# mazpie/genrl

Measured on AMD Instinct MI355X. Metric: world-model+imag update steps/sec (B32xL32x64x64x3), higher is better.
Workload: dtype f32 (storage, accumulation, every non-GEMM kernel and the fp32-MFMA GEMMs; the forward / dgrad / weight-gradient products of the imagination rollout, of the Dense+LN+SiLU chains from 192 rows up and of the encoder / decoder convolutions take fp32 operands pre-split into two fp16 planes of the scaled

## Files before the change

### genrl_amd/csrc/gemm_planes.hip

```cpp
#include "common.h"
#include "genrl_hip.h"
#include <type_traits>

typedef __bf16 bf16x8_t __attribute__((ext_vector_type(8)));
typedef _Float16 f16x8_t __attribute__((ext_vector_type(8)));
typedef unsigned u32x4 __attribute__((ext_vector_type(4)));

namespace {

struct PlaneSeg {
  const u16* a; long a_ld, a_plane;
  const u16* b; long b_ld, b_plane;
  int k;
  const float* a_inv; const float* b_inv;
};

struct SampleEpi {
  const float* q;
  long ldq;
  float* sample; long lds;
  u16* sp; long sld, splane; float* sinv;
  float a;
};

// ... 9 lines not shown
  float eps; int act;
  float* y; long ldy;
  u16* yp; long yld, yplane; float* yinv;
  float* mean; float* rstd;
  float* part;
  unsigned* sync;
};

struct PairSel {
  const u16* b; long b_ld, b_plane; const float* b_inv;
  float* C; long ldc; int N, accumulate;
  int tn0, nx;
};

__device__ __forceinline__ float pow2_ratio(float a, float b) {
  const int ea = (int)((__builtin_bit_cast(unsigned, a) >> 23) & 255u), eb = (int)((__builtin_bit_cast(unsigned, b) >> 23) & 255u);
  const int e = min(max(ea - eb + 127, 1), 254);
  return __builtin_bit_cast(float, (unsigned)e << 23);
}
__device__ __forceinline__ bool zero_row_inv(float inv) { return __builtin_bit_cast(unsigned, inv) == (4u << 23); }

__device__ __forceinline__ void glds16(const void* g, unsigned lds_byte_addr) {
  __builtin_amdgcn_global_load_lds((const __attribute__((address_space(1))) void*)g,
                                   (__attribute__((address_space(3))) void*)(uintptr_t)lds_byte_addr, 16, 0, 0);
}

template <int N> __device__ __forceinline__ void wait_vm() { asm volatile("s_waitcnt vmcnt(%0)" ::"i"(N) : "memory"); }

template <int TM, int TN, int BK, int NACC, int FMT, int NS, bool FOLD, bool CONV, int PF, bool LNE, bool IS_PAIR>
__device__ __forceinline__ void gemm_planes_body(PlaneSeg s0, PlaneSeg s1, float* __restrict__ C, long ldc,
                                                 const float* __restrict__ bias, int M, int N, int accumulate,
                                                 int tiles_m, int tiles_n, int xcd_m, SampleEpi smp, ConvGather cg, LnEpi ln, PairSel pr) {
  static_assert(!LNE || (TM * TN == 1 && FMT == 1 && !CONV && PF == 0), "LayerNorm epilogue: 64x64 h2 tile");
  static_assert(!IS_PAIR || (TM * TN == 1 && FMT == 1 && !CONV && PF == 0 && !LNE), "pair of products: 64x64 h2 tile");
  constexpr int BM = 64 * TM, BN = 64 * TN;
  static_assert(!(FMT == 1 && FOLD) || (BM == 64 && BN == 64), "segment fold: 64x64 h2 tile");
  constexpr int NPL = FMT ? 2 : 3, NPROD = FMT ? 3 : 6;
  constexpr int ROWB = BK * 2;
  constexpr int CPR = ROWB / 16;
  constexpr int RPC = 1024 / ROWB;
  constexpr int A_BYTES = NPL * BM * ROWB, B_BYTES = NPL * BN * ROWB, STAGE = A_BYTES + B_BYTES;
  constexpr int APIECES = A_BYTES / 1024, BPIECES = B_BYTES / 1024;
  static_assert(APIECES % 2 == 0 && BPIECES % 2 == 0, "pieces split over two waves per operand");
  constexpr int NPA = APIECES / 2, NPB = BPIECES / 2;
  constexpr int NPMAX = NPA > NPB ? NPA : NPB;
  constexpr int KS = BK / 16;
  static_assert(PF == 0 || (BK == 64 && !CONV), "prefetch: 128-byte tile rows, plain operands");
  constexpr int NPF = PF ? TM : 0;
  constexpr int EPI = FMT == 1 ? 4 * (BM + 2 * BN) : 0, EPI_AT = NS * STAGE + (PF ? 1024 : 0);
  constexpr int LN_AT = EPI_AT + EPI, LN_G = LN_AT, LN_B = LN_AT + 4096, LN_R = LN_AT + 8192, LN_U = LN_AT + 9216, LN_T = LN_AT + 9472, LN_BYTES = LNE ? 9728 : 0;
  __shared__ __attribute__((aligned(1024))) unsigned char lds[EPI_AT + EPI + LN_BYTES];

  int bid = blockIdx.x, tile_m, tile_n;
  {
    const int ntiles = tiles_m * tiles_n;
    int x = bid % 8;
    const int i = bid / 8;
    if constexpr (LNE) {
      unsigned xcc;
      asm volatile("s_getreg_b32 %0, hwreg(HW_REG_XCC_ID)" : "=s"(xcc));
      x = (int)(xcc & 7u);
      tile_n = i % tiles_n; tile_m = (i / tiles_n) * 8 + x;
      if (tile_m >= tiles_m) return;
    } else if (xcd_m > 0) {
      const int sub_m = tiles_m / xcd_m, sub_n = tiles_n / (8 / xcd_m);
      const int xm = x / (8 / xcd_m), xn = x % (8 / xcd_m);
      tile_m = xm * sub_m + i / sub_n;
      tile_n = xn * sub_n + i % sub_n;
    } else {
      const int q = ntiles / 8, r = ntiles % 8;
      bid = (x < r ? x * (q + 1) : r * (q + 1) + (x - r) * q) + i;
      tile_m = bid / tiles_n;
      tile_n = bid % tiles_n;
    }
  }
  if constexpr (IS_PAIR) {
    const int tn1 = tiles_n - pr.tn0;
    bool second;
    if (pr.nx > 0) {
      const int sub_n = tiles_n / pr.nx, q0 = pr.tn0 / pr.nx, xn = tile_n / sub_n, jn = tile_n % sub_n;
      second = jn >= q0;
      tile_n = second ? xn * (tn1 / pr.nx) + jn - q0 : xn * q0 + jn;
    } else {
      second = tile_n >= pr.tn0;
      if (second) tile_n -= pr.tn0;
    }
    if (second) {
      s0.b = pr.b; s0.b_ld = pr.b_ld; s0.b_plane = pr.b_plane; s0.b_inv = pr.b_inv;
      C = pr.C; ldc = pr.ldc; N = pr.N; accumulate = pr.accumulate;
    }
  }
  const int m0 = tile_m * BM, n0 = tile_n * BN;
  const int tid = threadIdx.x, lane = tid & 63;
  const int wave = __builtin_amdgcn_readfirstlane(tid >> 6);
  const int wm = wave >> 1, wn = wave & 1;
  const unsigned lds0 = (unsigned)(uintptr_t)lds;

  const bool isB = wave >= 2;
  const int npieces = isB ? NPB : NPA;
  const int rows_t = isB ? BN : BM;
  const int gpp = rows_t / RPC;
  const int r_in = lane / CPR, slot = lane % CPR;
  const char* gbase;
  unsigned voff[NPMAX];
  unsigned pfoff[NPF ? NPF : 1];
  auto setup = [&](const PlaneSeg& s) __attribute__((always_inline)) {
    const u16* P = isB ? s.b : s.a;
    const long ld = isB ? s.b_ld : s.a_ld, plane = isB ? s.b_plane : s.a_plane;
    const int rows_total = isB ? N : M, r0 = isB ? n0 : m0;
    gbase = reinterpret_cast<const char*>(P);
    if constexpr (PF > 0) {
#pragma unroll
      for (int i = 0; i < NPF; ++i) {
        const int L = ((wave & 1) * NPF + i) * 64 + lane;
        const int p = L / rows_t, row = L % rows_t;
        pfoff[i] = (unsigned)((p * plane + (long)min(r0 + row, rows_total - 1) * ld) * 2);
      }
    }
#pragma unroll
    for (int i = 0; i < NPMAX; ++i) {
      const int q = (wave & 1) * npieces + i;
      const int p = q / gpp, row = (q % gpp) * RPC + r_in;
      const int f = BK == 64 ? (row >> 1) & 7 : (row >> 2) & 3;
      voff[i] = (unsigned)((p * plane + (long)min(r0 + row, rows_total - 1) * ld) * 2 + ((slot ^ f) << 4));
    }
  };
  unsigned koff[2] = {0u, 0u};
  int kch[2] = {0, 0}, kkw[2] = {0, 0}, kkk[2] = {0, 0};
  if constexpr (CONV) {
    if (!isB) {
      const long ld = s0.a_ld, plane = s0.a_plane;
      gbase = reinterpret_cast<const char*>(s0.a);
#pragma unroll
      for (int i = 0; i < NPMAX; ++i) {
        const int q = (wave & 1) * npieces + i;
        const int p = q / gpp, row = (q % gpp) * RPC + r_in;
        const int m = min(m0 + row, M - 1);
        const int n_img = m / (cg.Ho * cg.Wo), rem = m - n_img * (cg.Ho * cg.Wo);
        const int oy = rem / cg.Wo, ox = rem - oy * cg.Wo;
        voff[i] = (unsigned)(((long)p * plane + ((long)(n_img * cg.H + cg.s * oy) * cg.W + cg.s * ox) * ld) * 2);
      }
#pragma unroll
      for (int par = 0; par < 2; ++par) {
        const int f = (4 * par + (r_in >> 1)) & 7;
        const int kk = 8 * (slot ^ f);
        const int tap = kk / cg.C, ch = kk - tap * cg.C, kh = tap / cg.k, kw = tap - kh * cg.k;
        kkk[par] = kk; kch[par] = ch; kkw[par] = kw;
        koff[par] = (unsigned)((((long)kh * cg.W + kw) * ld + ch) * 2);
      }
    }
  }
  const unsigned piece0 = lds0 + (isB ? A_BYTES : 0) + (wave & 1) * npieces * 1024;
  const int l32 = lane & 31, h32 = lane >> 5;
  const int f_rd = BK == 64 ? (l32 >> 1) & 7 : (l32 >> 2) & 3;
  unsigned xoff[KS];
#pragma unroll
  for (int s = 0; s < KS; ++s) xoff[s] = (unsigned)(((2 * s + h32) ^ f_rd) << 4);
  const unsigned a_row = lds0 + (wm * 32 * TM + l32) * ROWB, b_row = lds0 + A_BYTES + (wn * 32 * TN + l32) * ROWB;

  f32x16 acc[NACC][TM][TN];
#pragma unroll
  for (int c = 0; c < NACC; ++c)
#pragma unroll
    for (int i = 0; i < TM; ++i)
#pragma unroll
      for (int j = 0; j < TN; ++j)
#pragma unroll
        for (int r = 0; r < 16; ++r) acc[c][i][j][r] = 0.f;

  auto ldfrag = [&](unsigned addr) __attribute__((always_inline)) -> u32x4 {
    return *reinterpret_cast<const __attribute__((address_space(3))) u32x4*>((uintptr_t)addr);
  };
  constexpr int NB_ = TM + TN, NR = KS * NB_ * NPL, NM = KS * NPROD * TM * TN;
  constexpr int KB = 2;
  u32x4 fr[2][KS][NB_][NPL];
  unsigned a_s[KS], b_s[KS];
#pragma unroll
  for (int s = 0; s < KS; ++s) { a_s[s] = a_row + xoff[s]; b_s[s] = b_row + xoff[s]; }
  auto read_one = [&](int set, int r, int buf) __attribute__((always_inline)) {
    const int s = r / (NB_ * NPL), p = (r / NB_) % NPL, blk = r % NB_;
    fr[set][s][blk][p] = blk < TM ? ldfrag(a_s[s] + (p * (BM * ROWB) + blk * 32 * ROWB + buf * STAGE))
                                  : ldfrag(b_s[s] + (p * (BN * ROWB) + (blk - TM) * 32 * ROWB + buf * STAGE));
  };
  auto mfma_one = [&](int set, int m) __attribute__((always_inline)) {
    constexpr int PA[6] = {FMT ? 1 : 2, FMT ? 0 : 1, 0, 0, 1, 0}, PB[6] = {0, 0, FMT ? 1 : 2, 0, 1, 1};
// ... 3 lines not shown
    if constexpr (FMT == 0)
      c = __builtin_amdgcn_mfma_f32_32x32x16_bf16(__builtin_bit_cast(bf16x8_t, fr[set][s][TM + j][PB[t]]),
                                                  __builtin_bit_cast(bf16x8_t, fr[set][s][i][PA[t]]), c, 0, 0, 0);
    else
      c = __builtin_amdgcn_mfma_f32_32x32x16_f16(__builtin_bit_cast(f16x8_t, fr[set][s][TM + j][PB[t]]),
                                                 __builtin_bit_cast(f16x8_t, fr[set][s][i][PA[t]]), c, 0, 0, 0);
  };

  const float* const ainv_l = s1.k ? s1.a_inv : s0.a_inv;
  const float* const binv_l = s1.k ? s1.b_inv : s0.b_inv;
  if constexpr (FMT == 1) {
    const float* src = wave == 0 ? ainv_l : (wave == 1 ? binv_l : (wave == 2 ? bias : nullptr));
    const int base = wave == 0 ? m0 : n0, lim = (wave == 0 ? M : N) - 1, cnt = (wave == 0 ? BM : BN) / 64;
    const unsigned dst = lds0 + EPI_AT + (wave == 0 ? 0 : (wave == 1 ? 4 * BM : 4 * (BM + BN)));
    if (src) {
#pragma unroll
      for (int j = 0; j < (BM > BN ? BM : BN) / 64; ++j)
        if (j < cnt)
          __builtin_amdgcn_global_load_lds((const __attribute__((address_space(1))) void*)(src + min(base + 64 * j + lane, lim)),
                                           (__attribute__((address_space(3))) void*)(uintptr_t)(dst + 256 * j), 4, 0, 0);
    }
  }
  if constexpr (LNE) {
    const int f0 = min(256 * wave + 4 * lane, N - 4);
    __builtin_amdgcn_global_load_lds((const __attribute__((address_space(1))) void*)(ln.gamma + f0),
                                     (__attribute__((address_space(3))) void*)(uintptr_t)(lds0 + LN_G + 1024 * wave), 16, 0, 0);
    __builtin_amdgcn_global_load_lds((const __attribute__((address_space(1))) void*)(ln.beta + f0),
                                     (__attribute__((address_space(3))) void*)(uintptr_t)(lds0 + LN_B + 1024 * wave), 16, 0, 0);
    if (wave == 3)
      __builtin_amdgcn_global_load_lds((const __attribute__((address_space(1))) void*)(ln.part + ln_slab(tiles_n) + ((long)(tile_m * tiles_n + tile_n) * 64 + lane) * 4 + 1),
                                       (__attribute__((address_space(3))) void*)(uintptr_t)(lds0 + LN_T), 4, 0, 0);
  }
  const int nk0 = s0.k / BK, nk = nk0 + s1.k / BK;
  static_assert(NPA == NPB, "square wave grids only (one DMA count per wave)");
  constexpr int NP = NPA;
  if (!(CONV && !isB)) setup(s0);
  int seg_left = nk0, left = nk;
  bool first = true;
  auto next_stage = [&]() __attribute__((always_inline)) {
    if constexpr (CONV) {
      if (!isB) {
        if (!first && left > 0) {
          const unsigned ld2 = (unsigned)(s0.a_ld * 2);
#pragma unroll
          for (int par = 0; par < 2; ++par) {
            if (kkk[par] + 64 + 8 <= cg.K) {
              kkk[par] += 64;
              int ch = kch[par] + 64, kw = kkw[par];
              unsigned off = koff[par] + 128u;
#pragma unroll
              for (int rep = 0; rep < 2; ++rep)
                if (ch >= cg.C) {
                  ch -= cg.C; off -= (unsigned)(cg.C * 2);
                  ++kw; off += ld2;
                  if (kw == cg.k) { kw = 0; off += (unsigned)(cg.W - cg.k) * ld2; }
                }
              kch[par] = ch; kkw[par] = kw; koff[par] = off;
            }
          }
        }
        first = false;
        --seg_left; --left;
        return;
      }
    }
    if (seg_left == 0 && left > 0) { setup(s1); seg_left = left; }
    else if (!first && left > 0) gbase += BK * 2;
    first = false;
    --seg_left; --left;
  };
  auto prefetch = [&]() __attribute__((always_inline)) {
    if constexpr (PF > 0) {
      const int ahead = min(PF, max(seg_left, 0)) * (BK * 2);
#pragma unroll
      for (int i = 0; i < NPF; ++i)
        __builtin_amdgcn_global_load_lds((const __attribute__((address_space(1))) void*)(gbase + (size_t)pfoff[i] + ahead),
                                         (__attribute__((address_space(3))) void*)(uintptr_t)(lds0 + NS * STAGE + wave * 256), 4, 0, 0);
    }
  };
  auto issue_one = [&](int buf, int i) __attribute__((always_inline)) {
    if constexpr (CONV) {
      if (!isB) { glds16(gbase + (size_t)(voff[i] + koff[i & 1]), piece0 + buf * STAGE + i * 1024); return; }
    }
    glds16(gbase + (size_t)voff[i], piece0 + buf * STAGE + i * 1024);
  };
#pragma unroll
  for (int st = 0; st < NS; ++st) {
    next_stage();
    if (st) prefetch();
#pragma unroll
    for (int i = 0; i < NP; ++i) issue_one(st, i);
  }
  next_stage();
  wait_vm<(NS - 1) * (NP + NPF)>();
  __builtin_amdgcn_s_barrier();
#pragma unroll
  for (int r = 0; r < NR; ++r) read_one(0, r, 0);

  if constexpr (FMT == 1 && FOLD) {
    if (s1.k && wave < 2) {
      typedef __attribute__((address_space(3))) float lds_f32;
      lds_f32* const f = reinterpret_cast<lds_f32*>((uintptr_t)(lds0 + EPI_AT + 4 * (wave * BM + lane)));
      if ((wave ? s1.b_inv : s1.a_inv) && zero_row_inv(*f)) {
        const float* const inv0 = wave ? s0.b_inv : s0.a_inv;
        *f = inv0 ? inv0[min((wave ? n0 : m0) + lane, (wave ? N : M) - 1)] : 1.f;
      }
    }
  }
  auto epi1 = [&](int i) __attribute__((always_inline)) -> float {
    return *reinterpret_cast<const __attribute__((address_space(3))) float*>((uintptr_t)(lds0 + EPI_AT + 4 * i));
  };
  int it = 0;
  auto fold = [&]() __attribute__((always_inline)) {
    if constexpr (FMT == 1) {
#pragma unroll
      for (int i = 0; i < TM; ++i) {
        const int row = min(m0 + (wm * TM + i) * 32 + l32, M - 1);
        const int ri = (wm * TM + i) * 32 + l32;
        const float rf = (s0.a_inv && s1.a_inv) ? pow2_ratio(s0.a_inv[row], epi1(ri)) : (s0.a_inv ? s0.a_inv[row] : (s1.a_inv ? pow2_ratio(1.f, epi1(ri)) : 1.f));
#pragma unroll
        for (int j = 0; j < TN; ++j)
#pragma unroll
          for (int v = 0; v < 16; ++v) {
            const int col = min(n0 + (wn * TN + j) * 32 + 8 * (v / 4) + 4 * h32 + v % 4, N - 1);
            const int ci = BM + (wn * TN + j) * 32 + 8 * (v / 4) + 4 * h32 + v % 4;
            const float cf = (s0.b_inv && s1.b_inv) ? pow2_ratio(s0.b_inv[col], epi1(ci)) : (s0.b_inv ? s0.b_inv[col] : (s1.b_inv ? pow2_ratio(1.f, epi1(ci)) : 1.f));
#pragma unroll
            for (int c = 0; c < NACC; ++c) acc[c][i][j][v] *= rf * cf;
          }
      }
    }
  };

  constexpr int NSIDE = NP + NR;
  constexpr int PER = (NSIDE + 1) / 2 <= NM - KB - 2 ? 2 : 3;
  static_assert(NR >= 2 * NP, "side-op pattern: two reads per DMA");
  static_assert((NSIDE + PER - 1) / PER <= NM - KB - 2, "not enough MFMAs to hide the side operations");
  auto iteration = [&](auto SET, auto BUF) __attribute__((always_inline)) {
    constexpr int set = decltype(SET)::value, b0 = decltype(BUF)::value;
    constexpr int buf1 = (b0 + 1) % NS, buf3 = b0;
    if constexpr (FMT == 1 && FOLD) {
      if (it == nk0) fold();
    }
#pragma unroll
    for (int m = 0; m < KB; ++m) mfma_one(set, m);
    __builtin_amdgcn_sched_barrier(0);
    wait_vm<(NS - 2) * (NP + NPF)>();
    asm volatile("s_waitcnt lgkmcnt(0)" ::: "memory");
    __builtin_amdgcn_s_barrier();
    __builtin_amdgcn_sched_barrier(0);
    prefetch();
#pragma unroll
    for (int m = KB; m < NM; ++m) {
      mfma_one(set, m);
      const int lo = (m - KB) * PER, hi = lo + PER;
#pragma unroll
      for (int o = lo; o < hi; ++o) {
        if (o >= NSIDE) continue;
        if (o < 3 * NP && o % 3 == 2) {
          issue_one(buf3, o / 3);
        } else {
          read_one(1 - set, o < 3 * NP ? o - o / 3 : o - NP, buf1);
        }
      }
      __builtin_amdgcn_sched_barrier(0);
    }
    next_stage();
    ++it;
  };
  constexpr int PERIOD = NS % 2 ? 2 * NS : NS;
  auto run = [&](auto self, auto P, bool guarded) __attribute__((always_inline)) -> void {
    constexpr int p = decltype(P)::value;
    if constexpr (p < PERIOD) {
      if (guarded && it >= nk) return;
      iteration(std::integral_constant<int, p % 2>{}, std::integral_constant<int, p % NS>{});
      self(self, std::integral_constant<int, p + 1>{}, guarded);
    }
  };
  while (it + PERIOD <= nk) run(run, std::integral_constant<int, 0>{}, false);
  run(run, std::integral_constant<int, 0>{}, true);

  if constexpr (LNE) {
    typedef __attribute__((address_space(1))) unsigned gu32_;
    auto ldsf = [&](int byte_off) __attribute__((always_inline)) -> float {
      return *reinterpret_cast<const __attribute__((address_space(3))) float*>((uintptr_t)(lds0 + byte_off));
    };
    auto ldsw = [&](int byte_off, float v) __attribute__((always_inline)) {
      *reinterpret_cast<__attribute__((address_space(3))) float*>((uintptr_t)(lds0 + byte_off)) = v;
    };
    auto ldsf4 = [&](int byte_off) __attribute__((always_inline)) -> f32x4 {
      return *reinterpret_cast<const __attribute__((address_space(3))) f32x4*>((uintptr_t)(lds0 + byte_off));
    };
    const int rl = wm * 32 + l32, row = m0 + rl;
    const float ra = ainv_l ? ldsf(EPI_AT + 4 * rl) : 1.f;
    float o[16];
#pragma unroll
    for (int gq = 0; gq < 4; ++gq) {
      const int ci = wn * 32 + 8 * gq + 4 * h32;
      f32x4 cb = {1.f, 1.f, 1.f, 1.f}, bs = {0.f, 0.f, 0.f, 0.f};
      if (binv_l) cb = ldsf4(EPI_AT + 4 * (BM + ci));
      if (bias) bs = ldsf4(EPI_AT + 4 * (BM + BN + ci));
#pragma unroll
      for (int v = 0; v < 4; ++v) {
        const float lo = acc[0][0][0][4 * gq + v] + acc[2][0][0][4 * gq + v];
        o[4 * gq + v] = (lo * (1.f / 2048.f) + acc[1][0][0][4 * gq + v]) * ra * cb[v] + bs[v];
      }
    }
    float sm = 0.f;
#pragma unroll
    for (int v = 0; v < 16; ++v) sm += o[v];
    sm += __shfl_xor(sm, 32, 64);
    if (h32 == 0) ldsw(LN_R + 4 * (wave * 32 + l32), sm);
    __syncthreads();
// ... 1109 lines not shown
  for (int i = 0; i < n; ++i) {
    const int Co = d[i].transpose ? d[i].R : d[i].Cn;
    if (d[i].R <= 0 || d[i].Cn <= 0 || d[i].ld_out < Co || !d[i].inv || (d[i].ld_out & 63)) return GENRL_EINVAL;
  }
  hipStream_t s = (hipStream_t)stream;
  for (int pass = 0; pass < 2; ++pass) {
    int i = 0;
    while (i < n) {
      SplitBatch rows{}, cols{}, tiles{};
      int nb = 0;
      for (; i < n && nb < 32; ++i) {
        if ((d[i].transpose != 0) != (pass == 1)) continue;
        const SplitEntry e{d[i].src, d[i].ldx, d[i].R, d[i].Cn, d[i].out, d[i].ld_out, d[i].plane, d[i].inv};
        rows.e[nb] = cols.e[nb] = tiles.e[nb] = e;
        rows.blk0[nb + 1] = rows.blk0[nb] + cdiv(e.R, 4);
        cols.blk0[nb + 1] = cols.blk0[nb] + cdiv(e.Cn, 32);
        tiles.blk0[nb + 1] = tiles.blk0[nb] + cdiv(e.ld_out, 32) * cdiv(e.Cn, 32);
        ++nb;
      }
      if (!nb) continue;
      rows.n = cols.n = tiles.n = nb;
      if (pass == 0) {
        split_h2_rows_batch_kernel<<<rows.blk0[nb], 256, 0, s>>>(rows);
      } else {
        h2_colmax_batch_kernel<<<cols.blk0[nb], 256, 0, s>>>(cols);
        split_h2_t_batch_kernel<<<tiles.blk0[nb], 256, 0, s>>>(tiles);
      }
      GENRL_CHECK_LAUNCH();
    }
  }
  return GENRL_OK;
}

struct H2Route { bool big, two; };
static H2Route h2_route(int M, int N, int K, bool sample) {
  static const char* two_env = getenv("GENRL_PLANES_2PER");
  const long t64 = (long)cdiv(M, 64) * cdiv(N, 64);
  H2Route r;
  r.big = sample ? false : (g_planes_force_tile ? g_planes_force_tile == 2 : t64 >= 2048);
  r.two = !sample && (two_env ? two_env[0] == '1' : (t64 > 256 && K <= 1536));
  return r;
}

static int gemm_h2_impl(const uint16_t* a0, long a0_ld, long a0_plane, const float* a0_inv, const uint16_t* b0, long b0_ld, long b0_plane,
                        const float* b0_inv, int k0, const uint16_t* a1, long a1_ld, long a1_plane, const float* a1_inv,
                        const uint16_t* b1, long b1_ld, long b1_plane, const float* b1_inv, int k1,
                        float* C, long ldc, const float* bias, int M, int N, int accumulate, void* stream, const SampleEpi& smp) {
  GENRL_ENTER();
  if (M <= 0 || N <= 0 || k0 <= 0 || (k0 & 63) || (k1 & 63) || k1 < 0) return GENRL_EINVAL;
  if ((a0_ld & 7) || (b0_ld & 7) || (k1 && ((a1_ld & 7) || (b1_ld & 7)))) return GENRL_EINVAL;
  PlaneSeg s0{a0, a0_ld, a0_plane, b0, b0_ld, b0_plane, k0, a0_inv, b0_inv}, s1{a1, a1_ld, a1_plane, b1, b1_ld, b1_plane, k1, a1_inv, b1_inv};
  const H2Route rt = h2_route(M, N, k0 + k1, smp.q != nullptr);
  const bool big = rt.big;
  if (big && !g_planes_force_tile) {
    const int tm = cdiv(M, 128), tn = cdiv(N, 128), total = tm * tn, r = total % 256;
    if (total > 256 && r && r <= 128 && r % tn == 0 && (M & 127) == 0) {
      const int M1 = (tm - r / tn) * 128, M2 = M - M1;
      int rc = gemm_h2_impl(a0, a0_ld, a0_plane, a0_inv, b0, b0_ld, b0_plane, b0_inv, k0, a1, a1_ld, a1_plane, a1_inv, b1, b1_ld, b1_plane,
                            b1_inv, k1, C, ldc, bias, M1, N, accumulate, stream, smp);
      if (rc != GENRL_OK) return rc;
      return gemm_h2_impl(a0 + (long)M1 * a0_ld, a0_ld, a0_plane, a0_inv ? a0_inv + M1 : nullptr, b0, b0_ld, b0_plane, b0_inv, k0,
                          a1 ? a1 + (long)M1 * a1_ld : nullptr, a1_ld, a1_plane, a1_inv ? a1_inv + M1 : nullptr, b1, b1_ld, b1_plane, b1_inv, k1,
                          C + (long)M1 * ldc, ldc, bias, M2, N, accumulate, stream, smp);
    }
  }
  if (big) {
    const int tm = cdiv(M, 128), tn = cdiv(N, 128);
    const PlaneSeg none{nullptr, 0, 0, nullptr, 0, 0, 0, nullptr, nullptr};
    for (int seg = 0; seg < (k1 ? 2 : 1); ++seg) {
      const PlaneSeg& sg = seg ? s1 : s0;
      const float* bs = seg ? nullptr : bias;
      const int acc = seg ? 1 : accumulate;
      log_launch("h2/128", M, N, sg.k, kk_bytes(M, N, sg.k));
      route(!hl_on() ? GENRL_ROUTE_128_PLAIN : use_wide(N) ? GENRL_ROUTE_128_HLW : GENRL_ROUTE_128_HL);
      if (hl_on() && use_wide(N)) {
        const int tw = cdiv(N, 192);
        gemm_planes_hlw_kernel<false, 3><<<tm * tw, 256, 0, (hipStream_t)stream>>>(sg, C, ldc, bs, M, N, acc, tm, tw, xcd_split(tm, tw), ConvGather{});
      } else if (hl_on()) {
        gemm_planes_hl_kernel<false><<<tm * tn, 256, 0, (hipStream_t)stream>>>(sg, C, ldc, bs, M, N, acc, tm, tn, xcd_split(tm, tn) | (1 << 8), ConvGather{});
      } else
        gemm_planes_kernel<2, 2, 64, 2, 1, 2, false><<<tm * tn, 256, 0, (hipStream_t)stream>>>(sg, none, C, ldc, bs, M, N, acc, tm, tn,
                                                                                           xcd_split(tm, tn), SampleEpi{}, ConvGather{}, LnEpi{});
      GENRL_CHECK_LAUNCH();
    }
  } else {
    const int tm = cdiv(M, 64), tn = cdiv(N, 64);
    log_launch("h2/64", M, N, k0 + k1, kk_bytes(M, N, k0 + k1));
#define L64(NS_) gemm_planes_kernel<1, 1, 64, 3, 1, NS_, true><<<tm * tn, 256, 0, (hipStream_t)stream>>>( \
    s0, s1, C, ldc, bias, M, N, accumulate, tm, tn, xcd_split(tm, tn), smp, ConvGather{}, LnEpi{})
    const bool two = rt.two;
    route(smp.q ? GENRL_ROUTE_64_SAMPLE : (two ? GENRL_ROUTE_64_NS2 : GENRL_ROUTE_64_NS3));
    if (two) L64(2);
    else L64(3);
#undef L64
  }
  GENRL_CHECK_LAUNCH();
  return GENRL_OK;
}

int genrl_gemm_h2_conv(const uint16_t* img, long ld_img, long plane_img, const float* img_inv, int Nimg, int H, int W, int Cc, int k,
                       const uint16_t* b, long b_ld, long b_plane, const float* b_inv, float* C, long ldc, const float* bias, int N,
                       int accumulate, void* stream) {
  GENRL_ENTER();
  route_reset();
  const int Ho = (H - k) / 2 + 1, Wo = (W - k) / 2 + 1, K = k * k * Cc;
  const long Ml = (long)Nimg * Ho * Wo;
  if (Nimg <= 0 || Ho <= 0 || Wo <= 0 || N <= 0 || (Cc & 7) || Cc < 48 || ld_img < Cc || (ld_img & 7) || (b_ld & 63) || b_ld < K || b_ld >= K + 64 || K < 64 ||
      !img_inv || !b_inv || Ml > 0x7fffffffL)
    return GENRL_EINVAL;
  if ((((long)Nimg * H * W * ld_img + plane_img) * 2) >= 0xffffffffL) return GENRL_EINVAL;
  const int M = (int)Ml;
  PlaneSeg s0{img, ld_img, plane_img, b, b_ld, b_plane, (int)b_ld, img_inv, b_inv};
  const PlaneSeg none{nullptr, 0, 0, nullptr, 0, 0, 0, nullptr, nullptr};
  const bool wide = hl_on() && use_wide(N);
  const bool tall = hl_on() && use_tall96(N, K);
  const int tm = cdiv(M, tall ? 256 : 128), tn = tall ? 1 : cdiv(N, wide ? 192 : 128);
  log_launch("h2/conv128", M, N, (int)b_ld, 4.0 * ((double)Nimg * H * W * Cc + (double)N * b_ld + (double)M * N));
// ... 31 lines not shown
  const int M = (int)Ml;
  PlaneSeg s0{img, ld_img, plane_img, b, b_ld, b_plane, (int)b_ld, img_inv, b_inv};
  const bool wide = use_wide(N);
  const int tm = cdiv(M, 128), tn = cdiv(N, wide ? 192 : 128);
  log_launch("h2/subpixel128", M, N, (int)b_ld, 4.0 * ((double)Nimg * Hp * Wp * Cc + (double)N * b_ld + (double)Nimg * Ho * Wo * Co));
  route(wide ? GENRL_ROUTE_SUBPIXEL_HLW : GENRL_ROUTE_SUBPIXEL_HL);
  if (wide)
    gemm_planes_hlw_kernel<true, 3><<<tm * tn, 256, 0, (hipStream_t)stream>>>(s0, out, 4, bias, M, N, 0, tm, tn, xcd_split(tm, tn),
                                                                             ConvGather{Hp, Wp, Cc, T, Hq, Wq, K, 1, Ho, Wo, Co});
  else
    gemm_planes_hl_kernel<true><<<tm * tn, 256, 0, (hipStream_t)stream>>>(s0, out, 4, bias, M, N, 0, tm, tn, xcd_split(tm, tn),
                                                                          ConvGather{Hp, Wp, Cc, T, Hq, Wq, K, 1, Ho, Wo, Co});
  GENRL_CHECK_LAUNCH();
  return GENRL_OK;
}

int genrl_gemm_h2(const uint16_t* a0, long a0_ld, long a0_plane, const float* a0_inv, const uint16_t* b0, long b0_ld, long b0_plane,
                  const float* b0_inv, int k0, const uint16_t* a1, long a1_ld, long a1_plane, const float* a1_inv,
                  const uint16_t* b1, long b1_ld, long b1_plane, const float* b1_inv, int k1,
                  float* C, long ldc, const float* bias, int M, int N, int accumulate, void* stream) {
  route_reset();
  return gemm_h2_impl(a0, a0_ld, a0_plane, a0_inv, b0, b0_ld, b0_plane, b0_inv, k0, a1, a1_ld, a1_plane, a1_inv, b1, b1_ld, b1_plane,
                      b1_inv, k1, C, ldc, bias, M, N, accumulate, stream, SampleEpi{});
}

int genrl_gemm_h2_pair(const uint16_t* a, long a_ld, long a_plane, const float* a_inv, int k,
                       const uint16_t* b0, long b0_ld, long b0_plane, const float* b0_inv, float* C0, long ldc0, int N0, int accumulate0,
                       const uint16_t* b1, long b1_ld, long b1_plane, const float* b1_inv, float* C1, long ldc1, int N1, int accumulate1,
                       int M, void* stream) {
  GENRL_ENTER();
  route_reset();
  if (M <= 0 || N0 <= 0 || N1 <= 0 || k <= 0 || (k & 63) || (N0 & 63) || !a || !b0 || !b1 || !C0 || !C1) return GENRL_EINVAL;
  if ((a_ld & 7) || (b0_ld & 7) || (b1_ld & 7)) return GENRL_EINVAL;
  const int tm = cdiv(M, 64), tn0 = N0 / 64, tn1 = cdiv(N1, 64), tn = tn0 + tn1;
  for (int i = 0; i < 2; ++i) {
    const H2Route rt = h2_route(M, i ? N1 : N0, k, false);
    if (rt.big || rt.two) return GENRL_EINVAL;
  }
  const PlaneSeg s0{a, a_ld, a_plane, b0, b0_ld, b0_plane, k, a_inv, b0_inv};
  const int xm = xcd_split(tm, tn);
  const int nx = xm > 0 ? 8 / xm : 0;
  const PairSel pr{b1, b1_ld, b1_plane, b1_inv, C1, ldc1, N1, accumulate1, tn0, (nx > 0 && tn0 % nx == 0 && tn1 % nx == 0) ? nx : 0};
  log_launch("h2/64", M, (long)N0 + N1, k, kk_bytes(M, (long)N0 + N1, k));
  route(GENRL_ROUTE_64_NS3);
  gemm_planes_kernel<1, 1, 64, 3, 1, 3, PairOfProducts><<<tm * tn, 256, 0, (hipStream_t)stream>>>(s0, C0, ldc0, M, N0, accumulate0, tm, tn, xm, pr);
  GENRL_CHECK_LAUNCH();
  return GENRL_OK;
}

int genrl_gemm_h2_ln_ok(int M, int N) {
  if (M <= 0 || N <= 0 || (N & 63) || N > 1024) return 0;
  static int cus = -1;
  if (cus < 0) { int dev = 0, v = 0; if (hipGetDevice(&dev) != hipSuccess || hipDeviceGetAttribute(&v, hipDeviceAttributeMultiprocessorCount, dev) != hipSuccess) v = 0; cus = v; }
  if (cus < 256) return 0;
  const int tn = N / 64, tm = cdiv(M, 64);
  return tm <= 8 * (32 / tn) ? 1 : 0;
}
long genrl_gemm_h2_ln_part_floats(int M, int N) { (void)M; (void)N; return 16L * 65536; }
long genrl_gemm_h2_ln_sync_words(void) { return 32L; }
int genrl_gemm_h2_ln(const uint16_t* a0, long a0_ld, long a0_plane, const float* a0_inv, const uint16_t* b0, long b0_ld, long b0_plane,
                     const float* b0_inv, int k0, const uint16_t* a1, long a1_ld, long a1_plane, const float* a1_inv,
                     const uint16_t* b1, long b1_ld, long b1_plane, const float* b1_inv, int k1,
                     float* C, long ldc, const float* bias, int M, int N, const float* gamma, const float* beta, float eps, int act,
                     float* y, long ldy, float* mean, float* rstd, uint16_t* yp, long yld, long yplane, float* yinv,
                     float* part, unsigned* sync, void* stream) {
  GENRL_ENTER();
  route_reset();
  if (bad_act_code(act)) return GENRL_EINVAL;
  if (!genrl_gemm_h2_ln_ok(M, N) || k0 <= 0 || (k0 & 63) || (k1 & 63) || k1 < 0 || !gamma || !beta || !part || !sync || !C) return GENRL_EINVAL;
  if ((a0_ld & 7) || (b0_ld & 7) || (k1 && ((a1_ld & 7) || (b1_ld & 7))) || (ldc & 3) || (y && (ldy & 3)) || (yp && ((yld & 3) || !yinv))) return GENRL_EINVAL;
  if (((reinterpret_cast<uintptr_t>(C) | reinterpret_cast<uintptr_t>(bias) | reinterpret_cast<uintptr_t>(gamma) | reinterpret_cast<uintptr_t>(beta) |
        reinterpret_cast<uintptr_t>(y) | reinterpret_cast<uintptr_t>(part)) & 15) != 0 || (reinterpret_cast<uintptr_t>(yp) & 7) != 0)
    return GENRL_EINVAL;
  PlaneSeg s0{a0, a0_ld, a0_plane, b0, b0_ld, b0_plane, k0, a0_inv, b0_inv}, s1{a1, a1_ld, a1_plane, b1, b1_ld, b1_plane, k1, a1_inv, b1_inv};
  const int tm = cdiv(M, 64), tn = N / 64;
  const LnEpi ln{gamma, beta, eps, act, y, ldy, yp, yld, yplane, yinv, mean, rstd, part, sync};
  log_launch("h2/64ln", M, N, k0 + k1, kk_bytes(M, N, k0 + k1));
  route(GENRL_ROUTE_64_LN);
// ... 22 lines not shown
```

### include/genrl_hip.h

```cpp
#ifndef GENRL_HIP_H
#define GENRL_HIP_H
#include <stdint.h>
#ifdef __cplusplus
extern "C" {
#endif

long genrl_sgemm_ws_floats(int M, int N, int K);
int genrl_set_gemm_precision(int mode);
int genrl_sgemm_last_pipe(void);
int genrl_gemm_precision(void);
int genrl_sgemm(const float* A, long a_rs, long a_ks, const float* B, long b_rs, long b_ks, float* C, long ldc,
                const float* bias, int M, int N, int K, int accumulate, float* ws, long ws_floats, void* stream);

int genrl_sgemm_conv(const float* A, long a_rs, long a_ks, const float* B, long b_rs, long b_ks, float* C, long ldc,
                     const float* bias, int M, int N, int K, int accumulate, float* ws, long ws_floats, int which,
                     int img_h, int img_w, int img_c, int ksize, void* stream);

int genrl_split_h2(const float* x, long ldx, int R, int Cn, uint16_t* out, long ld_out, long plane, float* inv, int transpose,
                   void* stream);
int genrl_gemm_h2(const uint16_t* a0, long a0_ld, long a0_plane, const float* a0_inv, const uint16_t* b0, long b0_ld, long b0_plane,
                  const float* b0_inv, int k0, const uint16_t* a1, long a1_ld, long a1_plane, const float* a1_inv,
                  const uint16_t* b1, long b1_ld, long b1_plane, const float* b1_inv, int k1,
                  float* C, long ldc, const float* bias, int M, int N, int accumulate, void* stream);
int genrl_gemm_h2_pair(const uint16_t* a, long a_ld, long a_plane, const float* a_inv, int k,
// ... 126 lines not shown
int genrl_gemm_h2_tn_conv(const uint16_t* a, long a_ld, long a_plane, const float* a_inv, const uint16_t* img, long ld_img,
                          long plane_img, const float* img_inv, const unsigned* rowoff, int W, int Cc, int k, float* C, long ldc,
                          int NI, int M, int accumulate, void* ws, long ws_bytes, void* stream);
typedef struct {
  const float* src; long ldx; int R, Cn;
  uint16_t* out; long ld_out, plane; float* inv;
  int transpose;
} genrl_split_desc;
int genrl_split_h2_batch(const genrl_split_desc* descs, int n, void* stream);
int genrl_split_x3(const float* x, long ldx, int R, int Cn, uint16_t* out, long ld_out, long plane, int transpose,
                   void* stream);
int genrl_gemm_x3(const uint16_t* a0, long a0_ld, long a0_plane, const uint16_t* b0, long b0_ld, long b0_plane, int k0,
                  const uint16_t* a1, long a1_ld, long a1_plane, const uint16_t* b1, long b1_ld, long b1_plane, int k1,
                  float* C, long ldc, const float* bias, int M, int N, int accumulate, void* stream);
int genrl_planes_force_tile(int t);
long genrl_planes_last_route(void);
#define GENRL_ROUTE_64_NS3        0x1u
#define GENRL_ROUTE_64_NS2        0x2u
#define GENRL_ROUTE_64_SAMPLE     0x4u
#define GENRL_ROUTE_64_LN         0x8u
#define GENRL_ROUTE_128_PLAIN     0x10u
#define GENRL_ROUTE_128_HL        0x20u
#define GENRL_ROUTE_128_HLW       0x40u
#define GENRL_ROUTE_CONV_PLAIN    0x80u
#define GENRL_ROUTE_CONV_HL       0x100u
#define GENRL_ROUTE_CONV_HLW      0x200u
#define GENRL_ROUTE_CONV_TALL96   0x400u
#define GENRL_ROUTE_SUBPIXEL_HL   0x800u
#define GENRL_ROUTE_SUBPIXEL_HLW  0x1000u
#define GENRL_ROUTE_X3_64         0x2000u
#define GENRL_ROUTE_X3_128        0x4000u
#define GENRL_ROUTE_TN            0x8000u
#define GENRL_ROUTE_TN_CONV       0x10000u

int genrl_ln_act_fwd_h2(const float* x, long ldx, const float* gamma, const float* beta, float* y, long ldy, float* mean,
                        float* rstd, int M, int N, float eps, int act, uint16_t* yp, long ldp, long plane, float* inv,
                        void* stream);
typedef struct {
  const float* part; float* out0; float* out1; float* out2;
  int nchunk, N, np, accumulate;
} genrl_reduce_desc;
int genrl_ln_bwd_parts(int M, int N);
int genrl_reduce_params_batch(const genrl_reduce_desc* descs, int n, void* stream);
int genrl_ln_act_bwd_h2(const float* dy, long lddy, const float* x, long ldx, const float* gamma, const float* beta,
                        const float* mean, const float* rstd, float* dx, long lddx, float* dgamma, float* dbeta,
                        float* dcolsum, float* ws, int M, int N, int act, int accumulate_params, uint16_t* dxp, long ldp,
                        long plane, float* inv, void* stream);
int genrl_gru_gates_fwd_h2(const float* pre, const float* h, long ldh, const float* gamma, const float* beta,
                           float* hout, long ldo, float* hout2, const float* hout2_scale, float* mean, float* rstd,
                           int R, int D, float eps, uint16_t* hp, long ldp, long plane, float* inv, void* stream);
int genrl_gru_gates_bwd_h2(const float* dhout, long lddo, const float* dhout2, const float* dhout2_scale,
                           const float* pre, const float* h, long ldh, const float* gamma, const float* beta,
                           const float* mean, const float* rstd, float* dpre, float* dh, long lddh, float* dgamma,
                           float* dbeta, float* ws, int R, int D, int accumulate_params, const float* dhout2_parts,
                           int nparts, long part_stride, uint16_t* dprep, long ldp, long plane, float* inv, void* stream);
int genrl_actor_head_fwd_h2(const float* raw, const float* eps, float* action, float* mean, float* std, long R, int A,
                            float min_std, float max_std, long ld_action, uint16_t* ap, long ldp, long plane, float* inv,
                            void* stream);
int genrl_onehot_fwd_h2(const float* logits, const float* q, float* sample, float* probs, long G, int K, float unimix,
                        uint16_t* sp, int rowlen, long ldp, long plane, float* inv, void* stream);
int genrl_onehot_bwd_planes_only_ok(int K, int rowlen);
int genrl_onehot_bwd_h2(const float* logits, const float* gsample, float* dlogits, long G, int K, float unimix,
                        int accumulate, uint16_t* dp, int rowlen, long ldp, long plane, float* inv, void* stream);

int genrl_sgemm_skinny_parts(const float* A, long a_rs, const float* B, long b_rs, long b_ks, float* P, long ldp,
                             long part_stride, int M, int N, int K, int nparts, void* stream);
// ... 183 lines not shown
```

Before: 45.35.

## Add rectangular 64x192 and 128x64 h2 GEMM tiles for mid-size grids

Adds two rectangular tile shapes to the fp16-plane GEMM kernel. The 64x192 shape stages one plane per half-stage over four buffers, with a new half-iteration schedule. The 128x64 shape is also offered for the pair-of-products kernel. Routing picks them when the 64x64 tile count is over 256 but the rectangular tile count falls in 225-256, so the grid fits roughly one wave of CUs and each tile reuses more of its loaded operands. The cost is added kernel complexity, more register pressure, and a risk of scheduling or correctness issues in the new half-plane pipeline.

After: 45.91, median of 6. +1.2%, better.

```diff
diff --git a/genrl_amd/csrc/gemm_planes.hip b/genrl_amd/csrc/gemm_planes.hip
--- a/genrl_amd/csrc/gemm_planes.hip
+++ b/genrl_amd/csrc/gemm_planes.hip
@@ -65,18 +65,25 @@
                                                  const float* __restrict__ bias, int M, int N, int accumulate,
                                                  int tiles_m, int tiles_n, int xcd_m, SampleEpi smp, ConvGather cg, LnEpi ln, PairSel pr) {
   static_assert(!LNE || (TM * TN == 1 && FMT == 1 && !CONV && PF == 0), "LayerNorm epilogue: 64x64 h2 tile");
-  static_assert(!IS_PAIR || (TM * TN == 1 && FMT == 1 && !CONV && PF == 0 && !LNE), "pair of products: 64x64 h2 tile");
+  constexpr bool RECT = TM != TN;
+  static_assert(!RECT || (FMT == 1 && NACC == 3 && FOLD && !CONV && PF == 0 && !LNE && ((TM == 1 && TN == 3) || (TM == 2 && TN == 1))),
+                "rectangular tiles: 64x192 and 128x64, h2");
+  static_assert(!IS_PAIR || (TN == 1 && (TM == 1 || TM == 2) && FMT == 1 && !CONV && PF == 0 && !LNE), "pair of products: 64x64 or 128x64 h2 tile");
   constexpr int BM = 64 * TM, BN = 64 * TN;
-  static_assert(!(FMT == 1 && FOLD) || (BM == 64 && BN == 64), "segment fold: 64x64 h2 tile");
+  static_assert(!(FMT == 1 && FOLD) || (BM == 64 && BN == 64) || RECT, "segment fold: 64x64, 64x192 and 128x64 h2 tiles");
   constexpr int NPL = FMT ? 2 : 3, NPROD = FMT ? 3 : 6;
   constexpr int ROWB = BK * 2;
   constexpr int CPR = ROWB / 16;
   constexpr int RPC = 1024 / ROWB;
-  constexpr int A_BYTES = NPL * BM * ROWB, B_BYTES = NPL * BN * ROWB, STAGE = A_BYTES + B_BYTES;
+  constexpr bool HP = RECT && TN == 3;
+  static_assert(!HP || (BK == 64 && NS == 4), "64 x 192: four half stages of one plane of 64 k");
+  constexpr int NPLS = HP ? 1 : NPL;
+  constexpr int A_BYTES = NPLS * BM * ROWB, B_BYTES = NPLS * BN * ROWB, STAGE = A_BYTES + B_BYTES;
   constexpr int APIECES = A_BYTES / 1024, BPIECES = B_BYTES / 1024;
   static_assert(APIECES % 2 == 0 && BPIECES % 2 == 0, "pieces split over two waves per operand");
   constexpr int NPA = APIECES / 2, NPB = BPIECES / 2;
-  constexpr int NPMAX = NPA > NPB ? NPA : NPB;
+  static_assert(!RECT || (APIECES + BPIECES) % 4 == 0, "rectangular tiles: the stage's pieces divide over the four waves");
+  constexpr int NPMAX = RECT ? (APIECES + BPIECES) / 4 : (NPA > NPB ? NPA : NPB);
   constexpr int KS = BK / 16;
   static_assert(PF == 0 || (BK == 64 && !CONV), "prefetch: 128-byte tile rows, plain operands");
   constexpr int NPF = PF ? TM : 0;
@@ -135,6 +142,8 @@
   const int gpp = rows_t / RPC;
   const int r_in = lane / CPR, slot = lane % CPR;
   const char* gbase;
+  const char* gbase_b = nullptr;
+  long pl_a = 0, pl_b = 0;
   unsigned voff[NPMAX];
   unsigned pfoff[NPF ? NPF : 1];
   auto setup = [&](const PlaneSeg& s) __attribute__((always_inline)) {
@@ -142,6 +151,22 @@
     const long ld = isB ? s.b_ld : s.a_ld, plane = isB ? s.b_plane : s.a_plane;
     const int rows_total = isB ? N : M, r0 = isB ? n0 : m0;
     gbase = reinterpret_cast<const char*>(P);
+    if constexpr (RECT) {
+      gbase = reinterpret_cast<const char*>(s.a); gbase_b = reinterpret_cast<const char*>(s.b);
+      pl_a = s.a_plane * 2; pl_b = s.b_plane * 2;
+#pragma unroll
+      for (int i = 0; i < NPMAX; ++i) {
+        const int q = wave * NPMAX + i;
+        const bool pb = q >= APIECES;
+        const int qo = pb ? q - APIECES : q, gpo = (pb ? BN : BM) / RPC;
+        const int p = qo / gpo, row = (qo % gpo) * RPC + r_in;
+        const int f = BK == 64 ? (row >> 1) & 7 : (row >> 2) & 3;
+        const long ldo = pb ? s.b_ld : s.a_ld, plo = pb ? s.b_plane : s.a_plane;
+        const int last = (pb ? N : M) - 1, ro = pb ? n0 : m0;
+        voff[i] = (unsigned)((p * plo + (long)min(ro + row, last) * ldo) * 2 + ((slot ^ f) << 4));
+      }
+      return;
+    }
     if constexpr (PF > 0) {
 #pragma unroll
       for (int i = 0; i < NPF; ++i) {
@@ -183,7 +208,7 @@
       }
     }
   }
-  const unsigned piece0 = lds0 + (isB ? A_BYTES : 0) + (wave & 1) * npieces * 1024;
+  const unsigned piece0 = RECT ? lds0 + wave * NPMAX * 1024 : lds0 + (isB ? A_BYTES : 0) + (wave & 1) * npieces * 1024;
   const int l32 = lane & 31, h32 = lane >> 5;
   const int f_rd = BK == 64 ? (l32 >> 1) & 7 : (l32 >> 2) & 3;
   unsigned xoff[KS];
@@ -253,8 +278,8 @@
                                        (__attribute__((address_space(3))) void*)(uintptr_t)(lds0 + LN_T), 4, 0, 0);
   }
   const int nk0 = s0.k / BK, nk = nk0 + s1.k / BK;
-  static_assert(NPA == NPB, "square wave grids only (one DMA count per wave)");
-  constexpr int NP = NPA;
+  static_assert(RECT || NPA == NPB, "one DMA count per wave");
+  constexpr int NP = RECT ? NPMAX : NPA;
   if (!(CONV && !isB)) setup(s0);
   int seg_left = nk0, left = nk;
   bool first = true;
@@ -286,7 +311,10 @@
       }
     }
     if (seg_left == 0 && left > 0) { setup(s1); seg_left = left; }
-    else if (!first && left > 0) gbase += BK * 2;
+    else if (!first && left > 0) {
+      gbase += BK * 2;
+      if constexpr (RECT) gbase_b += BK * 2;
+    }
     first = false;
     --seg_left; --left;
   };
@@ -303,28 +331,64 @@
     if constexpr (CONV) {
       if (!isB) { glds16(gbase + (size_t)(voff[i] + koff[i & 1]), piece0 + buf * STAGE + i * 1024); return; }
     }
+    if constexpr (RECT) {
+      glds16((wave * NPMAX + i >= APIECES ? gbase_b : gbase) + (size_t)voff[i], piece0 + buf * STAGE + i * 1024);
+      return;
+    }
     glds16(gbase + (size_t)voff[i], piece0 + buf * STAGE + i * 1024);
   };
-#pragma unroll
-  for (int st = 0; st < NS; ++st) {
+  const int nu0 = 2 * nk0, nu = 2 * nk;
+  int hissued = 0;
+  auto next_half = [&]() __attribute__((always_inline)) {
+    if (hissued == nu0 && hissued < nu) setup(s1);
+    else if (hissued > 0 && hissued < nu) {
+      if (hissued & 1) { gbase += pl_a; gbase_b += pl_b; }
+      else { gbase += 128 - pl_a; gbase_b += 128 - pl_b; }
+    }
+    ++hissued;
+  };
+  auto read_half = [&](int set, int p, int r, int buf) __attribute__((always_inline)) {
+    const int s = r / NB_, blk = r % NB_;
+    fr[set][s][blk][p] = blk < TM ? ldfrag(a_s[s] + (blk * 32 * ROWB + buf * STAGE)) : ldfrag(b_s[s] + ((blk - TM) * 32 * ROWB + buf * STAGE));
+  };
+  if constexpr (HP) {
+#pragma unroll
+    for (int st = 0; st < NS; ++st) {
+      next_half();
+#pragma unroll
+      for (int i = 0; i < NP; ++i) issue_one(st, i);
+    }
+    next_half();
+    wait_vm<(NS - 1) * NP>();
+    __builtin_amdgcn_s_barrier();
+#pragma unroll
+    for (int r = 0; r < KS * NB_; ++r) read_half(0, 0, r, 0);
+  } else {
+#pragma unroll
+    for (int st = 0; st < NS; ++st) {
+      next_stage();
+      if (st) prefetch();
+#pragma unroll
+      for (int i = 0; i < NP; ++i) issue_one(st, i);
+    }
     next_stage();
-    if (st) prefetch();
-#pragma unroll
-    for (int i = 0; i < NP; ++i) issue_one(st, i);
-  }
-  next_stage();
-  wait_vm<(NS - 1) * (NP + NPF)>();
-  __builtin_amdgcn_s_barrier();
-#pragma unroll
-  for (int r = 0; r < NR; ++r) read_one(0, r, 0);
+    wait_vm<(NS - 1) * (NP + NPF)>();
+    __builtin_amdgcn_s_barrier();
+#pragma unroll
+    for (int r = 0; r < NR; ++r) read_one(0, r, 0);
+  }
 
   if constexpr (FMT == 1 && FOLD) {
     if (s1.k && wave < 2) {
       typedef __attribute__((address_space(3))) float lds_f32;
-      lds_f32* const f = reinterpret_cast<lds_f32*>((uintptr_t)(lds0 + EPI_AT + 4 * (wave * BM + lane)));
-      if ((wave ? s1.b_inv : s1.a_inv) && zero_row_inv(*f)) {
-        const float* const inv0 = wave ? s0.b_inv : s0.a_inv;
-        *f = inv0 ? inv0[min((wave ? n0 : m0) + lane, (wave ? N : M) - 1)] : 1.f;
+#pragma unroll
+      for (int j = 0; j < (BM > BN ? BM : BN) / 64; ++j) {
+        if (j >= (wave ? BN : BM) / 64) break;
+        lds_f32* const f = reinterpret_cast<lds_f32*>((uintptr_t)(lds0 + EPI_AT + 4 * (wave * BM + 64 * j + lane)));
+        if ((wave ? s1.b_inv : s1.a_inv) && zero_row_inv(*f)) {
+          const float* const inv0 = wave ? s0.b_inv : s0.a_inv;
+          *f = inv0 ? inv0[min((wave ? n0 : m0) + 64 * j + lane, (wave ? N : M) - 1)] : 1.f;
+        }
       }
     }
   }
@@ -334,21 +398,25 @@
   int it = 0;
   auto fold = [&]() __attribute__((always_inline)) {
     if constexpr (FMT == 1) {
+      int Mf = M, Nf = N;
+      if constexpr (TM * TN > 1) asm volatile("" : "+s"(Mf), "+s"(Nf));
 #pragma unroll
       for (int i = 0; i < TM; ++i) {
-        const int row = min(m0 + (wm * TM + i) * 32 + l32, M - 1);
+        const int row = min(m0 + (wm * TM + i) * 32 + l32, Mf - 1);
         const int ri = (wm * TM + i) * 32 + l32;
         const float rf = (s0.a_inv && s1.a_inv) ? pow2_ratio(s0.a_inv[row], epi1(ri)) : (s0.a_inv ? s0.a_inv[row] : (s1.a_inv ? pow2_ratio(1.f, epi1(ri)) : 1.f));
 #pragma unroll
-        for (int j = 0; j < TN; ++j)
+        for (int j = 0; j < TN; ++j) {
+          if constexpr (TM * TN > 1) __builtin_amdgcn_sched_barrier(0);
 #pragma unroll
           for (int v = 0; v < 16; ++v) {
-            const int col = min(n0 + (wn * TN + j) * 32 + 8 * (v / 4) + 4 * h32 + v % 4, N - 1);
+            const int col = min(n0 + (wn * TN + j) * 32 + 8 * (v / 4) + 4 * h32 + v % 4, Nf - 1);
             const int ci = BM + (wn * TN + j) * 32 + 8 * (v / 4) + 4 * h32 + v % 4;
             const float cf = (s0.b_inv && s1.b_inv) ? pow2_ratio(s0.b_inv[col], epi1(ci)) : (s0.b_inv ? s0.b_inv[col] : (s1.b_inv ? pow2_ratio(1.f, epi1(ci)) : 1.f));
 #pragma unroll
             for (int c = 0; c < NACC; ++c) acc[c][i][j][v] *= rf * cf;
           }
+        }
       }
     }
   };
@@ -398,8 +466,70 @@
       self(self, std::integral_constant<int, p + 1>{}, guarded);
     }
   };
-  while (it + PERIOD <= nk) run(run, std::integral_constant<int, 0>{}, false);
-  run(run, std::integral_constant<int, 0>{}, true);
+  int u = 0;
+  auto half_iter = [&](auto UC) __attribute__((always_inline)) {
+    constexpr int U = decltype(UC)::value;
+    constexpr bool LPH = (U & 1) != 0;
+    constexpr int HS = U >> 1;
+    constexpr int NMH = (LPH ? 2 : 1) * KS * TM * TN, NRH = KS * NB_, NSD = NRH + NP;
+    constexpr int PERH = (NSD + (NMH - KB) - 1) / (NMH - KB);
+    static_assert(U < 0 || (NRH == 2 * NP && PERH <= 3), "side-op pattern: read, read, DMA");
+    auto mfma_h = [&](int m) __attribute__((always_inline)) {
+      const int j = m % TN, i = (m / TN) % TM;
+      if constexpr (!LPH) {
+        const int s = m / (TM * TN);
+        acc[1][i][j] = __builtin_amdgcn_mfma_f32_32x32x16_f16(__builtin_bit_cast(f16x8_t, fr[HS][s][TM + j][0]), __builtin_bit_cast(f16x8_t, fr[HS][s][i][0]),
+                                                              acc[1][i][j], 0, 0, 0);
+      } else {
+        const int s = m / (2 * TM * TN), t = (m / (TM * TN)) % 2;
+        if (t == 0)
+          acc[0][i][j] = __builtin_amdgcn_mfma_f32_32x32x16_f16(__builtin_bit_cast(f16x8_t, fr[HS][s][TM + j][0]), __builtin_bit_cast(f16x8_t, fr[0][s][i][1]),
+                                                                acc[0][i][j], 0, 0, 0);
+        else
+          acc[2][i][j] = __builtin_amdgcn_mfma_f32_32x32x16_f16(__builtin_bit_cast(f16x8_t, fr[0][s][TM + j][1]), __builtin_bit_cast(f16x8_t, fr[HS][s][i][0]),
+                                                                acc[2][i][j], 0, 0, 0);
+      }
+    };
+    if constexpr (!LPH) {
+      if (u == nu0) fold();
+    }
+#pragma unroll
+    for (int m = 0; m < KB; ++m) mfma_h(m);
+    __builtin_amdgcn_sched_barrier(0);
+    wait_vm<(NS - 2) * NP>();
+    asm volatile("s_waitcnt lgkmcnt(0)" ::: "memory");
+    __builtin_amdgcn_s_barrier();
+    __builtin_amdgcn_sched_barrier(0);
+#pragma unroll
+    for (int m = KB; m < NMH; ++m) {
+      mfma_h(m);
+#pragma unroll
+      for (int o = (m - KB) * PERH; o < (m - KB + 1) * PERH; ++o) {
+        if (o >= NSD) continue;
+        if (o % 3 == 2) issue_one(U, o / 3);
+        else if constexpr (LPH) read_half(1 - HS, 0, o - o / 3, (U + 1) % NS);
+        else read_half(0, 1, o - o / 3, (U + 1) % NS);
+      }
+      __builtin_amdgcn_sched_barrier(0);
+    }
+    next_half();
+    ++u;
+  };
+  if constexpr (HP) {
+    while (u + 4 <= nu) {
+      half_iter(std::integral_constant<int, 0>{});
+      half_iter(std::integral_constant<int, 1>{});
+      half_iter(std::integral_constant<int, 2>{});
+      half_iter(std::integral_constant<int, 3>{});
+    }
+    if (u < nu) {
+      half_iter(std::integral_constant<int, 0>{});
+      half_iter(std::integral_constant<int, 1>{});
+    }
+  } else {
+    while (it + PERIOD <= nk) run(run, std::integral_constant<int, 0>{}, false);
+    run(run, std::integral_constant<int, 0>{}, true);
+  }
 
   if constexpr (LNE) {
     typedef __attribute__((address_space(1))) unsigned gu32_;
@@ -1575,13 +1705,26 @@
   return GENRL_OK;
 }
 
-struct H2Route { bool big, two; };
-static H2Route h2_route(int M, int N, int K, bool sample) {
+struct H2Route { bool big, two; int rect; };
+static int rect_env() {
+  static const int v = [] { const char* e = getenv("GENRL_PLANES_RECT"); return !e ? -1 : (e[0] == '0' ? 0 : (e[0] == '3' ? 3 : (e[0] == '4' ? 4 : -1))); }();
+  return v;
+}
+static H2Route h2_route(int M, int N, int K, bool sample, bool pair = false) {
   static const char* two_env = getenv("GENRL_PLANES_2PER");
   const long t64 = (long)cdiv(M, 64) * cdiv(N, 64);
   H2Route r;
   r.big = sample ? false : (g_planes_force_tile ? g_planes_force_tile == 2 : t64 >= 2048);
   r.two = !sample && (two_env ? two_env[0] == '1' : (t64 > 256 && K <= 1536));
+  r.rect = 0;
+  if (sample) return r;
+  if (g_planes_force_tile) {
+    if (g_planes_force_tile == 4 || (g_planes_force_tile == 3 && !pair)) r.rect = g_planes_force_tile;
+  } else if (!r.big && !r.two && t64 > 256 && rect_env() != 0) {
+    const long c192 = (long)cdiv(M, 64) * cdiv(N, 192), c128 = (long)cdiv(M, 128) * cdiv(N, 64);
+    if (!pair && rect_env() != 4 && c192 > 224 && c192 <= 256) r.rect = 3;
+    else if (rect_env() != 3 && c128 > 224 && c128 <= 256) r.rect = 4;
+  }
   return r;
 }
 
@@ -1626,6 +1769,17 @@
                                                                                            xcd_split(tm, tn), SampleEpi{}, ConvGather{}, LnEpi{});
       GENRL_CHECK_LAUNCH();
     }
+  } else if (rt.rect) {
+    const bool w = rt.rect == 3;
+    const int tm = cdiv(M, w ? 64 : 128), tn = cdiv(N, w ? 192 : 64);
+    log_launch("h2/rect", M, N, k0 + k1, kk_bytes(M, N, k0 + k1));
+    route(w ? GENRL_ROUTE_64X192 : GENRL_ROUTE_128X64);
+    if (w)
+      gemm_planes_kernel<1, 3, 64, 3, 1, 4, true><<<tm * tn, 256, 0, (hipStream_t)stream>>>(s0, s1, C, ldc, bias, M, N, accumulate, tm, tn, xcd_split(tm, tn),
+                                                                                          SampleEpi{}, ConvGather{}, LnEpi{});
+    else
+      gemm_planes_kernel<2, 1, 64, 3, 1, 3, true><<<tm * tn, 256, 0, (hipStream_t)stream>>>(s0, s1, C, ldc, bias, M, N, accumulate, tm, tn, xcd_split(tm, tn),
+                                                                                          SampleEpi{}, ConvGather{}, LnEpi{});
   } else {
     const int tm = cdiv(M, 64), tn = cdiv(N, 64);
     log_launch("h2/64", M, N, k0 + k1, kk_bytes(M, N, k0 + k1));
@@ -1723,18 +1877,22 @@
   route_reset();
   if (M <= 0 || N0 <= 0 || N1 <= 0 || k <= 0 || (k & 63) || (N0 & 63) || !a || !b0 || !b1 || !C0 || !C1) return GENRL_EINVAL;
   if ((a_ld & 7) || (b0_ld & 7) || (b1_ld & 7)) return GENRL_EINVAL;
-  const int tm = cdiv(M, 64), tn0 = N0 / 64, tn1 = cdiv(N1, 64), tn = tn0 + tn1;
+  int tm = cdiv(M, 64);
+  const int tn0 = N0 / 64, tn1 = cdiv(N1, 64), tn = tn0 + tn1;
   for (int i = 0; i < 2; ++i) {
     const H2Route rt = h2_route(M, i ? N1 : N0, k, false);
     if (rt.big || rt.two) return GENRL_EINVAL;
   }
   const PlaneSeg s0{a, a_ld, a_plane, b0, b0_ld, b0_plane, k, a_inv, b0_inv};
+  const bool rect = (long)N0 + N1 <= 0x7fffffffL && h2_route(M, N0 + N1, k, false, true).rect == 4;
+  if (rect) tm = cdiv(M, 128);
   const int xm = xcd_split(tm, tn);
   const int nx = xm > 0 ? 8 / xm : 0;
   const PairSel pr{b1, b1_ld, b1_plane, b1_inv, C1, ldc1, N1, accumulate1, tn0, (nx > 0 && tn0 % nx == 0 && tn1 % nx == 0) ? nx : 0};
-  log_launch("h2/64", M, (long)N0 + N1, k, kk_bytes(M, (long)N0 + N1, k));
-  route(GENRL_ROUTE_64_NS3);
-  gemm_planes_kernel<1, 1, 64, 3, 1, 3, PairOfProducts><<<tm * tn, 256, 0, (hipStream_t)stream>>>(s0, C0, ldc0, M, N0, accumulate0, tm, tn, xm, pr);
+  log_launch(rect ? "h2/rect" : "h2/64", M, (long)N0 + N1, k, kk_bytes(M, (long)N0 + N1, k));
+  route(rect ? GENRL_ROUTE_128X64 : GENRL_ROUTE_64_NS3);
+  if (rect) gemm_planes_kernel<2, 1, 64, 3, 1, 3, PairOfProducts><<<tm * tn, 256, 0, (hipStream_t)stream>>>(s0, C0, ldc0, M, N0, accumulate0, tm, tn, xm, pr);
+  else gemm_planes_kernel<1, 1, 64, 3, 1, 3, PairOfProducts><<<tm * tn, 256, 0, (hipStream_t)stream>>>(s0, C0, ldc0, M, N0, accumulate0, tm, tn, xm, pr);
   GENRL_CHECK_LAUNCH();
   return GENRL_OK;
 }
diff --git a/include/genrl_hip.h b/include/genrl_hip.h
--- a/include/genrl_hip.h
+++ b/include/genrl_hip.h
@@ -182,6 +182,8 @@
 #define GENRL_ROUTE_X3_128        0x4000u
 #define GENRL_ROUTE_TN            0x8000u
 #define GENRL_ROUTE_TN_CONV       0x10000u
+#define GENRL_ROUTE_64X192        0x20000u
+#define GENRL_ROUTE_128X64        0x40000u
 
 int genrl_ln_act_fwd_h2(const float* x, long ldx, const float* gamma, const float* beta, float* y, long ldy, float* mean,
                         float* rstd, int M, int N, float eps, int act, uint16_t* yp, long ldp, long plane, float* inv,
```
